# adaptivegenome/openge

Hardware: AMD Instinct MI355X
Metric: Mreads/sec sort+dedup (and realign intervals/sec), 1/2/4/8 MI355X (higher is better)
Workload: dtype u8

## Files before the change

include/openge_hip.h:

```cpp
#ifndef OPENGE_HIP_H
#define OPENGE_HIP_H

#include <stddef.h>
#include <stdint.h>

#ifdef __cplusplus
extern "C" {
#endif

typedef enum oge_status {
    OGE_OK = 0,
    OGE_ERR_ARG = -1,
    OGE_ERR_HIP = -2,
    OGE_ERR_LIMIT = -3,
    OGE_ERR_IO = -4
} oge_status;

typedef struct oge_ctx oge_ctx;

int oge_ctx_create(int device, oge_ctx **out);
int oge_device_count(void);
int oge_ctx_set_stream(oge_ctx *ctx, void *stream);
void *oge_ctx_stream(oge_ctx *ctx);
int oge_ctx_sync(oge_ctx *ctx);
// ... 87 lines not shown
                          uint64_t *n_dup_total);
int oge_bgzf_decode_shard(oge_comm *comm, const uint8_t *d_z, uint64_t zbytes, uint64_t own_bytes, const uint8_t **d_recs,
                          const uint64_t **d_off, uint64_t *n, uint8_t *hdr_out, uint64_t hdr_cap, uint64_t *hdr_len);
int oge_mergesort_bgzf_shard(oge_comm *comm, const uint8_t *d_z, uint64_t zbytes, uint64_t own_bytes, const oge_mergesort_opts *o,
                             const uint8_t **d_out, uint64_t *out_bytes, uint64_t *n_reads_total, uint64_t *n_dup_total);
int oge_synth_offsets_range_dev(oge_ctx *ctx, const void *params, uint64_t slot0, uint64_t nslots, uint64_t *d_offs);
int oge_synth_records_range_dev(oge_ctx *ctx, const void *params, uint64_t slot0, uint64_t nslots,
                                const uint64_t *d_offs, uint8_t *d_out);

typedef struct oge_realign_scan_batch {
    const uint8_t *cons;
    uint64_t cons_bytes;
    const uint64_t *cons_off;
    uint32_t n_cons;
    uint32_t n_reads;
    const uint8_t *bases;
    const uint8_t *quals;
    uint64_t read_bytes;
    const uint64_t *read_off;
    const int32_t *pairs;
    uint64_t n_pairs;
} oge_realign_scan_batch;
int oge_realign_scan(oge_ctx *ctx, const oge_realign_scan_batch *batch, int32_t *best_index, int32_t *best_score);

typedef struct oge_realign_opts {
    double lod_threshold;
    double mismatch_threshold;
    int32_t max_records_in_memory;
    int32_t max_isize_for_movement;
    int32_t max_pos_move_allowed;
    int32_t max_reads;
    int32_t no_original_alignment_tags;
    int32_t threads;
} oge_realign_opts;
void oge_realign_opts_init(oge_realign_opts *opts);

typedef struct oge_realign_result oge_realign_result;
int oge_localrealign(oge_ctx *ctx, const char *header_text, uint64_t header_len, const uint8_t *recs,
                     const uint64_t *rec_off, uint64_t n, const char *fasta_path, const char *intervals_path,
                     const oge_realign_opts *opts, oge_realign_result **out);
int oge_localrealign_multi(oge_ctx *const *ctxs, int n_ctx, const char *header_text, uint64_t header_len, const uint8_t *recs,
                           const uint64_t *rec_off, uint64_t n, const char *fasta_path, const char *intervals_path,
                           const oge_realign_opts *opts, oge_realign_result **out);
uint64_t oge_realign_result_count(const oge_realign_result *r);
const uint8_t *oge_realign_result_records(const oge_realign_result *r, uint64_t *bytes_out);
const uint64_t *oge_realign_result_offsets(const oge_realign_result *r);
const char *oge_realign_result_stats(const oge_realign_result *r);
void oge_realign_result_free(oge_realign_result *r);

int oge_synth_finalize(void *params);
uint64_t oge_synth_params_size(void);
int oge_synth_offsets_host(const void *params, uint64_t *offs, int threads);
int oge_synth_records_host(const void *params, const uint64_t *offs, uint8_t *out, int threads);
int oge_synth_header_text(const void *params, char *buf, uint64_t cap, uint64_t *len_out);
typedef struct oge_realign_synth_params {
    uint64_t seed;
    uint32_t n_ref, n_intervals, spacing, read_len, frags_per_interval;
    uint32_t qual_min, qual_max, ins_min, ins_max;
    uint32_t err_ppm, noindel_ppm, gapped_ppm, alt_indel_ppm, dup_ppm, mapq0_ppm, clip_ppm;
    uint32_t lower_ppm, n_ppm, md_ppm, uq_ppm;
} oge_realign_synth_params;
void oge_realign_synth_defaults(oge_realign_synth_params *p);
int oge_synth_realign(const oge_realign_synth_params *p, const char *fasta_path, const char *intervals_path,
                      const char *bam_path, int level, int threads);
int oge_synth_offsets_dev(oge_ctx *ctx, const void *params, uint64_t *d_offs);
int oge_synth_records_dev(oge_ctx *ctx, const void *params, const uint64_t *d_offs, uint8_t *d_out);

typedef struct oge_bam oge_bam;
int oge_bam_read(const char *path, int threads, oge_bam **out);
void oge_bam_free(oge_bam *b);
uint64_t oge_bam_count(const oge_bam *b);
const uint8_t *oge_bam_records(const oge_bam *b, uint64_t *bytes_out);
const uint64_t *oge_bam_offsets(const oge_bam *b);
int32_t oge_bam_n_ref(const oge_bam *b);
int oge_bam_header_text(const oge_bam *b, char *buf, uint64_t cap, uint64_t *len_out);
int oge_bam_markdup_opts(const oge_bam *b, oge_markdup_opts *opts, char **rg_ids_buf, int16_t **rg_lib_buf);
int oge_bam_write(const char *path, const char *header_text, uint64_t header_len, int sort_order,
                  const uint8_t *recs, const uint64_t *offs, uint64_t n, const uint32_t *order,
                  const uint16_t *flags, int level, int threads);

uint64_t oge_bgzf_bound(uint64_t n);
int oge_bgzf_deflate_dev(oge_ctx *ctx, const uint8_t *d_src, uint64_t n, int level, uint8_t *d_dst,
                         uint64_t dst_cap, uint64_t *out_bytes);
int oge_bgzf_deflate(oge_ctx *ctx, const uint8_t *src, uint64_t n, int level, uint8_t *dst, uint64_t dst_cap,
                     uint64_t *out_bytes);
enum { OGE_DEFL_FAST = 0, OGE_DEFL_NEAR = 1, OGE_DEFL_SPAN = 2 };
int oge_ctx_set_deflate_search(oge_ctx *ctx, int search);
int oge_ctx_deflate_search(oge_ctx *ctx);
int oge_bgzf_index(const uint8_t *z, uint64_t zbytes, uint64_t *d0, uint64_t *d1, uint64_t *uoff, uint32_t *crc,
                   uint64_t cap, uint64_t *nblk);
int oge_bgzf_index_dev(oge_ctx *ctx, const uint8_t *d_z, uint64_t zbytes, uint64_t *d_d0, uint64_t *d_d1,
                       uint64_t *d_uoff, uint32_t *d_crc, uint64_t cap, uint64_t *nblk);
int oge_bgzf_inflate_dev(oge_ctx *ctx, const uint8_t *d_z, uint64_t zbytes, const uint64_t *d_d0, const uint64_t *d_d1,
                         const uint64_t *d_uoff, const uint32_t *d_crc, uint64_t nblk, uint8_t *d_out);
uint64_t oge_infl_plan(uint64_t nblk, uint64_t lanes, uint64_t budget, uint64_t max_per_lane, int balanced,
                       uint64_t *sizes, uint64_t cap);
int oge_bgzf_inflate(oge_ctx *ctx, const uint8_t *z, uint64_t zbytes, uint8_t *out, uint64_t out_cap,
                     uint64_t *out_bytes);
int oge_bam_record_offsets_dev(oge_ctx *ctx, const uint8_t *d_stream, uint64_t rec_base, uint64_t end, int32_t n_ref,
                               uint64_t *d_off, uint64_t cap, uint64_t *n_out);
int oge_fix_bins_dev(oge_ctx *ctx, uint8_t *d_recs, const uint64_t *d_off, uint64_t n);
int oge_drop_flagged_dev(oge_ctx *ctx, const uint8_t *d_recs, const uint64_t *d_off, uint64_t n, uint16_t flag_mask,
                         uint8_t *d_out, uint64_t *d_out_off, uint64_t *n_out);

int oge_bai_build_dev(oge_ctx *ctx, const uint8_t *d_recs, const uint64_t *d_off, uint64_t n, int32_t n_ref,
                      uint64_t stream_base, const uint64_t *d_uoff, const uint64_t *d_cstart, uint64_t nblk,
                      const uint8_t **d_bai, uint64_t *bai_bytes);
int oge_bai_build(oge_ctx *ctx, const uint8_t *recs, uint64_t rec_bytes, const uint64_t *rec_off, uint64_t n,
                  int32_t n_ref, uint64_t stream_base, const uint64_t *uoff, const uint64_t *cstart, uint64_t nblk,
                  uint8_t *out, uint64_t cap, uint64_t *bai_bytes);
int oge_bam_index_dev(oge_ctx *ctx, const uint8_t *d_z, uint64_t zbytes, const uint8_t **d_bai, uint64_t *bai_bytes);
int oge_ctx_last_bai(oge_ctx *ctx, const uint8_t **d_bai, uint64_t *bai_bytes);

typedef struct oge_bai oge_bai;
int oge_bai_open(oge_ctx *ctx, const uint8_t *bai, uint64_t bytes, int32_t n_ref_expected, oge_bai **out);
void oge_bai_close(oge_bai *bai);
struct oge_region;
int oge_bai_query_dev(oge_ctx *ctx, const oge_bai *bai, const struct oge_region *regions, uint64_t n_regions, int32_t widen,
                      const uint64_t **d_ranges, uint64_t *n_ranges);
int oge_bai_query(oge_ctx *ctx, const oge_bai *bai, const struct oge_region *regions, uint64_t n_regions, int32_t widen,
                  uint64_t *out, uint64_t cap, uint64_t *n_ranges);
int oge_bam_decode_ranges_dev(oge_ctx *ctx, const uint8_t *d_z, uint64_t zbytes, const uint64_t *span_z,
                              const uint64_t *span_file, uint64_t n_spans, const uint64_t *d_ranges, uint64_t n_ranges,
                              int32_t n_ref, uint8_t **d_recs, uint64_t **d_off, uint64_t *n, uint64_t *rec_bytes);

typedef struct oge_bam_stats {
    uint64_t reads, mapped, forward, reverse, failed_qc, duplicates, paired, proper_pair, read1, read2, both_mapped,
        singletons;
    int32_t sorted;
    int32_t pad0;
    uint64_t n_insert, insert_sum, insert_mid_lo, insert_mid_hi;
    uint64_t n_lengths;
} oge_bam_stats;
enum { OGE_STATS_INSERTS = 1, OGE_STATS_LENGTHS = 2 };
int oge_stats_dev(oge_ctx *ctx, const uint8_t *d_recs, const uint64_t *d_off, uint64_t n, uint32_t want,
                  oge_bam_stats *stats, const uint32_t **d_len, const uint64_t **d_len_count);
int oge_stats(oge_ctx *ctx, const uint8_t *recs, uint64_t rec_bytes, const uint64_t *rec_off, uint64_t n, uint32_t want,
              oge_bam_stats *stats, uint32_t *len_out, uint64_t *len_count_out, uint64_t cap);
int oge_coverage_layout(int32_t n_ref, const int32_t *ref_len, int32_t binsize, uint64_t *base);
int oge_coverage_dev(oge_ctx *ctx, const uint8_t *d_recs, const uint64_t *d_off, uint64_t n, int32_t n_ref,
                     const int32_t *ref_len, int32_t binsize, const uint32_t **d_bins, uint64_t *n_skipped,
                     int32_t *overflow);
int oge_coverage(oge_ctx *ctx, const uint8_t *recs, uint64_t rec_bytes, const uint64_t *rec_off, uint64_t n,
                 int32_t n_ref, const int32_t *ref_len, int32_t binsize, uint32_t *bins_out, uint64_t cap,
                 uint64_t *n_skipped, int32_t *overflow);
int oge_bam_stats_dev(oge_ctx *ctx, const uint8_t *d_z, uint64_t zbytes, uint32_t want, oge_bam_stats *stats,
                      const uint32_t **d_len, const uint64_t **d_len_count);
int oge_bam_coverage_dev(oge_ctx *ctx, const uint8_t *d_z, uint64_t zbytes, int32_t binsize, const uint32_t **d_bins,
                         uint64_t *n_bins, uint64_t *n_skipped, int32_t *overflow);
int oge_bam_count_dev(oge_ctx *ctx, const uint8_t *d_z, uint64_t zbytes, uint64_t *n_reads);
int oge_ctx_last_refs(oge_ctx *ctx, int32_t *n_ref, const char **names, uint64_t *names_bytes, const int32_t **ref_len);

typedef struct oge_compare_region {
    int32_t left_ref, left_pos, right_ref, right_pos;
} oge_compare_region;
typedef struct oge_compare_result {
    uint64_t n_ref, n_other, common, additions, deletions, diff_entries, hard_runs;
} oge_compare_result;
enum { OGE_COMPARE_DIFF = 1 };
int oge_compare_dev(oge_ctx *ctx, const uint8_t *d_recs_a, const uint64_t *d_off_a, uint64_t n_a, const uint8_t *d_recs_b,
                    const uint64_t *d_off_b, uint64_t n_b, int32_t n_ref, const oge_compare_region *region, uint32_t want,
                    int debug_hash_bits, oge_compare_result *result, const uint8_t **d_diff, uint64_t *diff_bytes);
int oge_compare(oge_ctx *ctx, const uint8_t *recs_a, uint64_t rec_bytes_a, const uint64_t *rec_off_a, uint64_t n_a,
                const uint8_t *recs_b, uint64_t rec_bytes_b, const uint64_t *rec_off_b, uint64_t n_b, int32_t n_ref,
                const oge_compare_region *region, uint32_t want, int debug_hash_bits, oge_compare_result *result,
                uint8_t *diff_out, uint64_t cap, uint64_t *diff_bytes);
// ... 59 lines not shown
```

openge_amd/csrc/bgzf.hip:

```cpp
#include <hip/hip_runtime.h>

#include <cstdint>
#include <cstdlib>
#include <cstring>
#include <string>
#include <vector>

#include "bam_layout.h"
#include "oge_ctx.h"
#include "records.h"
#include "bgzf_dev.h"

namespace {

using namespace oge_bgzf;
constexpr int kT = 512;
constexpr int kSeg = 64;
constexpr int kSub = kT * kSeg;
constexpr int kNSub = 2;
constexpr int kNSeg = kT * kNSub;
constexpr int kHashBits = 12;
constexpr int kLit = 286, kDist = 30, kCl = 19;
constexpr int kFreq = kLit + kDist;
constexpr int kHdrWords = 144;
// ... 1093 lines not shown
            for (int b = 0; b < 4; ++b)
                if (s0 + 4 * k + b < len) v |= (uint32_t)s[s0 + 4 * k + b] << (8 * b);
            w[k] = v;
        }
    }
}

#ifndef OGE_EMIT_MPRE
#define OGE_EMIT_MPRE 8
#endif
constexpr int kMPre = OGE_EMIT_MPRE;
__device__ __forceinline__ void seg_tokens(const uint32_t *mp, uint32_t nm, uint32_t (&m)[kMPre]) {
    const uint32_t last = nm ? nm - 1 : 0;
#pragma unroll
    for (int k = 0; k < kMPre; ++k) m[k] = mp[(uint64_t)min((uint32_t)k, last) * kNSeg];
}

__device__ __forceinline__ uint32_t seg_bits(const uint32_t (&w)[16], uint64_t lm, uint32_t nm, const uint32_t *mp,
                                             const uint32_t (&m)[kMPre], const uint32_t *ct, const uint32_t *dist) {
    uint32_t bits = 0;
#pragma unroll
    for (int g = 0; g < 4; ++g) {
        uint32_t c[16];
#pragma unroll
        for (int i = 0; i < 16; ++i) c[i] = ct[(w[4 * g + (i >> 2)] >> (8 * (i & 3))) & 0xff];
#pragma unroll
        for (int i = 0; i < 16; ++i) bits += (lm >> (16 * g + i)) & 1 ? c[i] >> 24 : 0u;
    }
#pragma unroll
    for (int k = 0; k < kMPre; ++k)
        if ((uint32_t)k < nm) bits += match_bits(m[k], ct, dist);
    for (uint32_t k = kMPre; k < nm; ++k) bits += match_bits(mp[(uint64_t)k * kNSeg], ct, dist);
    return bits;
}

__device__ __forceinline__ void seg_emit(const uint32_t (&w)[16], uint64_t lm, uint32_t nm, const uint32_t *mp,
                                         uint32_t (&m)[kMPre], const uint32_t *ct, const uint32_t *dist, uint32_t *img,
                                         uint32_t bit) {
    uint32_t k = 0, cur = m[0], moff = nm ? (cur >> 23) : 64u;
    uint32_t lc, dv, dn;
    auto look = [&](uint32_t tok) {
        lc = ct[256 + ((tok >> 15) & 255)];
        dist_bits((tok & 0x7fff) + 1, dist, dv, dn);
    };
    look(cur);
    LdsBits bw;
    bw.init(img, bit);
#pragma unroll
    for (int g = 0; g < 4; ++g) {
        uint32_t c[16];
#pragma unroll
        for (int i = 0; i < 16; ++i) c[i] = ct[(w[4 * g + (i >> 2)] >> (8 * (i & 3))) & 0xff];
#pragma unroll
        for (int i0 = 0; i0 < 16; i0 += 2) {
            const int i = 16 * g + i0;
            const uint32_t a = (lm >> i) & 1 ? c[i0] : 0u, b = (lm >> (i + 1)) & 1 ? c[i0 + 1] : 0u;
            bw.put((a & 0xffffff) | ((b & 0xffffff) << (a >> 24)), (a >> 24) + (b >> 24));
            if (((uint32_t)i | 1u) == (moff | 1u)) {
#if OGE_EXP == 8
                ++k;
#pragma unroll
                for (int q = 0; q + 1 < kMPre; ++q) m[q] = m[q + 1];
                moff = k < nm && k < (uint32_t)kMPre ? m[0] >> 23 : 64u;
#else
                bw.put(lc & 0xffffff, lc >> 24);
                bw.put(dv, dn);
                ++k;
#pragma unroll
                for (int q = 0; q + 1 < kMPre; ++q) m[q] = m[q + 1];
                if (k < nm) {
                    cur = k < (uint32_t)kMPre ? m[0] : mp[(uint64_t)k * kNSeg];
                    moff = cur >> 23;
                    look(cur);
                } else {
                    moff = 64;
                }
#endif
            }
        }
    }
    bw.finish();
}

__global__ void __launch_bounds__(kT, 4) k_defl_emit(const uint8_t *__restrict__ src, uint64_t n, uint64_t blk0,
                                                     const uint64_t *__restrict__ lmask, const uint8_t *__restrict__ nmatch,
                                                     const uint32_t *__restrict__ mlist, const DeflTab *__restrict__ tabs,
                                                     const uint32_t *__restrict__ zpow, const uint32_t *__restrict__ offs,
                                                     const uint64_t *__restrict__ cbase, uint8_t *__restrict__ dst) {
    __shared__ __align__(16) uint32_t img[kSlot / 4 + 4];
    __shared__ uint32_t ct[512], dist[kDist];
    __shared__ uint32_t scan[kNSeg];
    __shared__ uint32_t wsum[kT / 64];
    __shared__ uint32_t crctab[4][256];
    __shared__ uint32_t zp[17][32];
    __shared__ uint32_t zl[32][16];
    __shared__ uint32_t crcs[kT / 64];
    __shared__ uint32_t sh_crc;
    const int t = threadIdx.x, lane = t & 63, wv = t >> 6;
    const uint64_t blk = blk0 + blockIdx.x;
    const uint64_t start = blk * kPay;
    const uint32_t len = (uint32_t)min<uint64_t>(kPay, n - start);
    const uint8_t *s = src + start;
    const DeflTab &T = tabs[blockIdx.x];
    const uint32_t total = T.total, stored = T.stored, hb = T.hdr_bits;
    for (int i = t; i < 512; i += kT) ct[i] = ct_entry(i, T.lit);
    for (int i = t; i < kDist; i += kT) dist[i] = T.dist[i];
    crc_setup<kT>(crctab, zp, zpow, t);
    for (int i = t; i < 32 * 16; i += kT) zl[i >> 4][i & 15] = zpow[17 * 32 + i];
    for (uint32_t i = t; i < (total + 15) / 16; i += kT) ((uint4 *)img)[i] = make_uint4(0, 0, 0, 0);
    __syncthreads();
    {
        const uint32_t c = crc_global512x4l(s, len, crctab, zl, zp, crcs, t);
        if (t == 0) sh_crc = c;
    }
    const uint32_t bsize = total - 1;
    if (stored) {
        for (uint32_t i = t; i < len; i += kT) ((uint8_t *)img)[23 + i] = s[i];
    } else {
        const uint32_t s0a = t * kSeg, s0b = kSub + t * kSeg;
        const uint64_t sga = (uint64_t)blockIdx.x * kNSeg + t, sgb = sga + kT;
        const uint64_t lma = s0a < len ? lmask[sga] : 0, lmb = s0b < len ? lmask[sgb] : 0;
        const uint32_t nma = s0a < len ? nmatch[sga] : 0, nmb = s0b < len ? nmatch[sgb] : 0;
        const uint32_t *mpa = mlist + ((uint64_t)blockIdx.x * kMaxM) * kNSeg + t, *mpb = mpa + kT;
        uint32_t ca, cb;
        {
            uint32_t w[16], m[kMPre];
            seg_load(s, s0a, len, w);
            seg_tokens(mpa, nma, m);
            ca = seg_bits(w, lma, nma, mpa, m, ct, dist);
            seg_load(s, s0b, len, w);
            seg_tokens(mpb, nmb, m);
            cb = seg_bits(w, lmb, nmb, mpb, m, ct, dist);
        }
        scan[t] = ca;
        scan[kT + t] = cb;
        __syncthreads();
        {
            const uint32_t a = scan[2 * t], b = scan[2 * t + 1];
            uint32_t x = a + b, inc = x;
#pragma unroll
            for (int o = 1; o < 64; o <<= 1) {
                const uint32_t y = __shfl_up(inc, o);
                if (lane >= o) inc += y;
            }
            if (lane == 63) wsum[wv] = inc;
            __syncthreads();
            uint32_t pre = 0;
            for (int q = 0; q < wv; ++q) pre += wsum[q];
            const uint32_t ex = pre + inc - x;
            __syncthreads();
            scan[2 * t] = ex;
            scan[2 * t + 1] = ex + a;
        }
        __syncthreads();
        for (uint32_t i = t; i < (hb + 31) / 32; i += kT) {
            const uint32_t v = T.hdr[i];
            atomicOr(img + 4 + i, v << 16);
            if (v >> 16) atomicOr(img + 5 + i, v >> 16);
        }
        {
            uint32_t w[16], m[kMPre];
            if (ca) {
                seg_load(s, s0a, len, w);
                seg_tokens(mpa, nma, m);
                seg_emit(w, lma, nma, mpa, m, ct, dist, img, 144 + hb + scan[t]);
            }
            if (cb) {
                seg_load(s, s0b, len, w);
                seg_tokens(mpb, nmb, m);
                seg_emit(w, lmb, nmb, mpb, m, ct, dist, img, 144 + hb + scan[kT + t]);
            }
        }
        if (t == kT - 1) {
            const uint32_t body_end = 144 + hb + scan[kNSeg - 1] + cb;
            LdsBits bw;
            bw.init(img, body_end);
            const uint32_t c = T.lit[256];
            bw.put(c & 0xffff, c >> 16);
            bw.finish();
        }
    }
    __syncthreads();
    uint8_t *ib = (uint8_t *)img;
    if (t == 0) {
        img[0] = 0x04088b1fu;
        img[1] = 0;
        img[2] = 0x0006ff00u;
        img[3] = 0x00024342u;
        ib[16] = (uint8_t)bsize, ib[17] = (uint8_t)(bsize >> 8);
        if (stored) {
            ib[18] = 1;
            ib[19] = (uint8_t)len, ib[20] = (uint8_t)(len >> 8);
            ib[21] = (uint8_t)~len, ib[22] = (uint8_t)(~len >> 8);
        }
        const uint32_t q = total - 8;
        for (int b = 0; b < 4; ++b) ib[q + b] = (uint8_t)(sh_crc >> (8 * b)), ib[q + 4 + b] = (uint8_t)(len >> (8 * b));
    }
    __syncthreads();
    uint8_t *D = dst + *cbase + offs[blockIdx.x];
    const uint32_t sh = (uint32_t)((uintptr_t)D & 3);
    OGE_G uint32_t *A = (OGE_G uint32_t *)((uintptr_t)D & ~(uintptr_t)3);
    const uint32_t nwords = (total + sh + 3) / 4;
    for (uint32_t g = t; g < nwords; g += kT) {
        const int32_t r0 = (int32_t)(4 * g) - (int32_t)sh;
        if (r0 >= 0 && r0 + 4 <= (int32_t)total) {
            A[g] = ld32(img, (uint32_t)r0);
        } else {
            for (int i = 0; i < 4; ++i) {
                const int32_t r = r0 + i;
                if (r >= 0 && r < (int32_t)total) ((OGE_G uint8_t *)(A + g))[i] = ib[r];
            }
        }
    }
}

constexpr uint32_t kMaxChunk = 16384, kPer = kMaxChunk / 1024;
__global__ void __launch_bounds__(1024) k_scan_chunk(const uint32_t *__restrict__ in, uint32_t n, uint32_t *__restrict__ out) {
    __shared__ uint32_t ws[16];
    const uint32_t t = threadIdx.x, lane = t & 63, w = t >> 6;
    uint32_t a[kPer], v = 0;
#pragma unroll
    for (uint32_t i = 0; i < kPer; ++i) {
        a[i] = kPer * t + i < n ? in[kPer * t + i] : 0;
        v += a[i];
    }
    uint32_t x = v;
#pragma unroll
    for (int d = 1; d < 64; d <<= 1) {
        const uint32_t y = __shfl_up(x, d, 64);
        if (lane >= (uint32_t)d) x += y;
    }
    if (lane == 63) ws[w] = x;
    __syncthreads();
    if (t < 16) {
        uint32_t s = ws[t], z = s;
        for (int d = 1; d < 16; d <<= 1) {
            const uint32_t y = __shfl_up(z, d, 16);
            if ((t & 15) >= (uint32_t)d) z += y;
        }
        ws[t] = z - s;
    }
    __syncthreads();
    uint32_t excl = ws[w] + x - v;
#pragma unroll
    for (uint32_t i = 0; i < kPer; ++i) {
        if (kPer * t + i < n) out[kPer * t + i] = excl;
        excl += a[i];
    }
}

__global__ void k_defl_advance(uint64_t *base, uint64_t *cbase, const uint32_t *offs, const uint32_t *sizes, uint32_t nb) {
    if (threadIdx.x == 0 && blockIdx.x == 0) {
        const uint64_t b = *base;
        *cbase = b;
        *base = b + (uint64_t)offs[nb - 1] + sizes[nb - 1];
    }
}

__global__ void k_fix_bins(uint8_t *__restrict__ recs, const uint64_t *__restrict__ off, uint64_t n) {
    const uint64_t i = (uint64_t)blockIdx.x * blockDim.x + threadIdx.x;
    if (i >= n) return;
    uint8_t *r = recs + off[i];
    oge_wr_u16(r + OGE_OFF_BIN, oge_rec_bin(r));
}

}


extern "C" uint64_t oge_bgzf_bound(uint64_t n) { return ((n + kPay - 1) / kPay) * (uint64_t)kSlot; }

extern "C" int oge_bgzf_deflate_dev(oge_ctx *ctx, const uint8_t *d_src, uint64_t n, int level, uint8_t *d_dst,
                                    uint64_t dst_cap, uint64_t *out_bytes) {
    if (!ctx) return oge_fail(nullptr, OGE_ERR_ARG, "null ctx");
    if (!out_bytes || (n && (!d_src || !d_dst))) return oge_fail(ctx, OGE_ERR_ARG, "null buffer");
    if (level < 0 || level > 9) return oge_fail(ctx, OGE_ERR_ARG, "level must be 0..9");
    const int depth = level >= 9 ? 32 : level == 8 ? 8 : 1, lazy = level >= 8 ? 1 : 0;
    const int search = level == 0 ? OGE_DEFL_FAST : ctx->deflate_search;
    if (dst_cap < oge_bgzf_bound(n)) return oge_fail(ctx, OGE_ERR_ARG, "dst_cap < oge_bgzf_bound(n)");
    OgeCall call(ctx, false);
    *out_bytes = 0;
    if (!n) return OGE_OK;
    const uint64_t nblk = (n + kPay - 1) / kPay;
    const int ncu = ctx->cu_count();
#ifndef OGE_DEFL_STREAMS
#define OGE_DEFL_STREAMS 3
#endif
#ifndef OGE_DEFL_CHUNK
#define OGE_DEFL_CHUNK kMaxChunk
#endif
    static_assert(OGE_DEFL_CHUNK <= kMaxChunk, "k_scan_chunk bound");
    constexpr uint64_t kPerPay = (uint64_t)kNSeg * 8 + kNSeg + (uint64_t)kMaxM * kNSeg * 4 + kFreq * 4 + sizeof(DeflTab) + 8;
    const int S0 = nblk > 4096 ? OGE_DEFL_STREAMS : 1;
    uint64_t chunk = std::min<uint64_t>(nblk, OGE_DEFL_CHUNK);
    if (chunk > 4096) {
        size_t fr = 0, tot = 0;
        if (hipMemGetInfo(&fr, &tot) != hipSuccess) fr = 0;
        uint64_t held = 0;
        for (int s = 0; s < 3; ++s) {
            const auto it = ctx->bufs.find("defl_mlist" + std::to_string(s));
            if (it != ctx->bufs.end()) held += it->second.cap / ((uint64_t)kMaxM * kNSeg * 4) * kPerPay;
        }
        while (chunk > 4096 && (uint64_t)S0 * chunk * kPerPay > (fr + held) / 4) chunk = std::max<uint64_t>(4096, chunk / 2);
    }
    static_assert(OGE_DEFL_STREAMS >= 1 && OGE_DEFL_STREAMS <= 3, "deflate: 1-3 streams");
    const int S = nblk > chunk ? OGE_DEFL_STREAMS : 1;
    struct Bufs {
        uint64_t *lmask, *cbase;
        uint32_t *mlist, *freq, *sizes, *offs;
        uint8_t *nmatch;
        DeflTab *tabs;
        hipStream_t st;
    } B[3];
    for (int s = 0; s < S; ++s) {
        const std::string x = std::to_string(s);
        B[s].lmask = (uint64_t *)ctx->ws(("defl_lmask" + x).c_str(), chunk * kNSeg * 8);
        B[s].nmatch = (uint8_t *)ctx->ws(("defl_nmatch" + x).c_str(), chunk * kNSeg);
        B[s].mlist = (uint32_t *)ctx->ws(("defl_mlist" + x).c_str(), chunk * kMaxM * kNSeg * 4);
        B[s].freq = (uint32_t *)ctx->ws(("defl_freq" + x).c_str(), chunk * kFreq * 4);
        B[s].tabs = (DeflTab *)ctx->ws(("defl_tabs" + x).c_str(), chunk * sizeof(DeflTab));
        B[s].sizes = (uint32_t *)ctx->ws(("defl_sizes" + x).c_str(), chunk * 4 + 16);
        B[s].offs = (uint32_t *)ctx->ws(("defl_offs" + x).c_str(), chunk * 4 + 16);
        B[s].cbase = (uint64_t *)ctx->ws(("defl_cbase" + x).c_str(), 16);
        B[s].st = S == 1 ? ctx->stream : ctx->side_stream(s);
        if (!B[s].lmask || !B[s].nmatch || !B[s].mlist || !B[s].freq || !B[s].tabs || !B[s].sizes || !B[s].offs ||
            !B[s].cbase || !B[s].st)
            return OGE_ERR_HIP;
    }
    uint32_t *zpow = (uint32_t *)ctx->ws("defl_zpow", (17 * 32 + 32 * 16) * 4);
    uint64_t *base = (uint64_t *)ctx->ws("defl_base", 16);
    if (!zpow || !base) return OGE_ERR_HIP;
    static struct {
        uint32_t z[17][32], zl[32][16];
    } zh = [] {
        decltype(zh) v;
        crc_zpow(v.z);
        crc_zlane<16>(v.z, 128, &v.zl[0][0]);
        return v;
    }();
    OGE_HIP_TRY(ctx, hipMemcpyAsync(zpow, &zh, sizeof(zh), hipMemcpyHostToDevice, ctx->stream));
    OGE_HIP_TRY(ctx, hipMemsetAsync(base, 0, 8, ctx->stream));
    OgeStage stage(ctx, "bgzf_deflate");
    hipEvent_t ev[4];
    for (auto &e : ev) OGE_HIP_TRY(ctx, hipEventCreateWithFlags(&e, hipEventDisableTiming));
    struct Evs {
        hipEvent_t *e;
        ~Evs() {
            for (int i = 0; i < 4; ++i) hipEventDestroy(e[i]);
        }
    } evs{ev};
    OGE_HIP_TRY(ctx, hipEventRecord(ev[3], ctx->stream));
    for (int s = 0; s < S; ++s)
        if (B[s].st != ctx->stream) OGE_HIP_TRY(ctx, hipStreamWaitEvent(B[s].st, ev[3], 0));
    uint64_t k = 0;
    for (uint64_t b0 = 0; b0 < nblk; b0 += chunk, ++k) {
        const uint32_t nb = (uint32_t)std::min(chunk, nblk - b0);
        Bufs &u = B[k % S];
        const uint32_t pg = (uint32_t)std::min<uint64_t>(nb, (uint64_t)ncu);
#define OGE_PARSE_X(C, N, S) \
    k_defl_parse_x<C, N, S><<<pg, kTP, 0, u.st>>>(d_src, n, b0, nb, u.lmask, u.nmatch, u.mlist, u.freq, depth, lazy)
        if (search == OGE_DEFL_FAST && depth > 1)
            k_defl_parse<true><<<pg, kTP, 0, u.st>>>(d_src, n, b0, nb, u.lmask, u.nmatch, u.mlist, u.freq, depth, lazy);
        else if (search == OGE_DEFL_FAST)
            k_defl_parse<false><<<pg, kTP, 0, u.st>>>(d_src, n, b0, nb, u.lmask, u.nmatch, u.mlist, u.freq, 1, 0);
        else if (search == OGE_DEFL_NEAR)
            depth > 1 ? OGE_PARSE_X(true, true, false) : OGE_PARSE_X(false, true, false);
        else if (search == OGE_DEFL_SPAN)
            depth > 1 ? OGE_PARSE_X(true, false, true) : OGE_PARSE_X(false, false, true);
        else
            depth > 1 ? OGE_PARSE_X(true, true, true) : OGE_PARSE_X(false, true, true);
#undef OGE_PARSE_X
        OGE_LAUNCH_CHECK(ctx);
        k_defl_huff<<<nb, 64, 0, u.st>>>(u.freq, u.tabs, n, b0, level, u.sizes);
        OGE_LAUNCH_CHECK(ctx);
        k_scan_chunk<<<1, 1024, 0, u.st>>>(u.sizes, nb, u.offs);
        OGE_LAUNCH_CHECK(ctx);
        if (k) OGE_HIP_TRY(ctx, hipStreamWaitEvent(u.st, ev[(k - 1) % S], 0));
        k_defl_advance<<<1, 64, 0, u.st>>>(base, u.cbase, u.offs, u.sizes, nb);
        OGE_LAUNCH_CHECK(ctx);
        OGE_HIP_TRY(ctx, hipEventRecord(ev[k % S], u.st));
        k_defl_emit<<<nb, kT, 0, u.st>>>(d_src, n, b0, u.lmask, u.nmatch, u.mlist, u.tabs, zpow, u.offs, u.cbase, d_dst);
        OGE_LAUNCH_CHECK(ctx);
    }
    if (S > 1) {
        for (int s = 0; s < S; ++s) {
            OGE_HIP_TRY(ctx, hipEventRecord(ev[s], B[s].st));
            OGE_HIP_TRY(ctx, hipStreamWaitEvent(ctx->stream, ev[s], 0));
        }
    }
    stage.end();
    uint64_t total = 0;
    OGE_HIP_TRY(ctx, hipMemcpyAsync(&total, base, 8, hipMemcpyDeviceToHost, ctx->stream));
    OGE_HIP_TRY(ctx, hipStreamSynchronize(ctx->stream));
    *out_bytes = total;
    return OGE_OK;
}

extern "C" int oge_bgzf_deflate(oge_ctx *ctx, const uint8_t *src, uint64_t n, int level, uint8_t *dst, uint64_t dst_cap,
                                uint64_t *out_bytes) {
    if (!ctx) return oge_fail(nullptr, OGE_ERR_ARG, "null ctx");
    if (!out_bytes || (n && (!src || !dst))) return oge_fail(ctx, OGE_ERR_ARG, "null buffer");
    hipSetDevice(ctx->device);
    *out_bytes = 0;
    if (!n) return OGE_OK;
    const uint64_t bound = oge_bgzf_bound(n);
    uint8_t *ds = (uint8_t *)ctx->ws("defl_hsrc", n + 16);
    uint8_t *dd = (uint8_t *)ctx->ws("defl_hdst", bound);
    if (!ds || !dd) return OGE_ERR_HIP;
    OGE_HIP_TRY(ctx, hipMemcpyAsync(ds, src, n, hipMemcpyHostToDevice, ctx->stream));
    uint64_t got = 0;
    int rc = oge_bgzf_deflate_dev(ctx, ds, n, level, dd, bound, &got);
    if (rc) return rc;
    if (got > dst_cap) return oge_fail(ctx, OGE_ERR_ARG, "dst_cap too small for the compressed stream");
    OGE_HIP_TRY(ctx, hipMemcpyAsync(dst, dd, got, hipMemcpyDeviceToHost, ctx->stream));
    OGE_HIP_TRY(ctx, hipStreamSynchronize(ctx->stream));
    *out_bytes = got;
    return OGE_OK;
}

extern "C" int oge_fix_bins_dev(oge_ctx *ctx, uint8_t *d_recs, const uint64_t *d_off, uint64_t n) {
    if (!ctx) return oge_fail(nullptr, OGE_ERR_ARG, "null ctx");
    hipSetDevice(ctx->device);
    if (!n) return OGE_OK;
    k_fix_bins<<<oge_ceil_div(n, 256), 256, 0, ctx->stream>>>(d_recs, d_off, n);
    OGE_LAUNCH_CHECK(ctx);
    return OGE_OK;
}
```

openge_amd/lib.py:

```python
from __future__ import annotations

import contextlib
import ctypes as C
import os
from pathlib import Path

import numpy as np

PKG = Path(__file__).resolve().parent
LIB_PATH = Path(os.environ["OGE_LIB"]) if os.environ.get("OGE_LIB") else PKG / "libopenge_hip.so"

MAX_REF = 64
DEFLATE_SEARCH = ("fast", "near", "span", "near+span")


class SynthParams(C.Structure):

    _fields_ = [
        ("seed", C.c_uint64), ("n_pairs", C.c_uint64), ("n_ref", C.c_uint32), ("read_len", C.c_uint32),
        ("ins_min", C.c_uint32), ("ins_max", C.c_uint32), ("dup_ppm", C.c_uint32), ("inter_ppm", C.c_uint32),
        ("munmap_ppm", C.c_uint32), ("clip_ppm", C.c_uint32), ("n_rg", C.c_uint32), ("qual_min", C.c_uint32),
        ("qual_max", C.c_uint32), ("shuffle", C.c_uint32),
        ("ref_len", C.c_uint64 * MAX_REF), ("ref_cum", C.c_uint64 * (MAX_REF + 1)),
    ]
# ... 182 lines not shown
    L = C.CDLL(str(LIB_PATH))
    vp, u64, i32, u32 = C.c_void_p, C.c_uint64, C.c_int32, C.c_uint32
    sig = {
        "oge_ctx_create": (C.c_int, [C.c_int, C.POINTER(vp)]),
        "oge_ctx_set_stream": (C.c_int, [vp, vp]),
        "oge_ctx_stream": (vp, [vp]),
        "oge_ctx_sync": (C.c_int, [vp]),
        "oge_ctx_destroy": (None, [vp]),
        "oge_last_error": (C.c_char_p, [vp]),
        "oge_ctx_timing": (C.c_int, [vp, C.c_char_p, C.POINTER(C.c_double)]),
        "oge_ctx_counter": (C.c_int, [vp, C.c_char_p, C.POINTER(u64)]),
        "oge_mergesort_reserve": (C.c_int, [vp, u64, C.POINTER(vp), C.POINTER(vp), C.POINTER(u64)]),
        "oge_version": (C.c_char_p, []),
        "oge_sort_coord": (C.c_int, [vp, vp, u64, vp, u64, i32, vp]),
        "oge_sort_coord_dev": (C.c_int, [vp, vp, vp, u64, i32, vp]),
        "oge_gather_records_dev": (C.c_int, [vp, vp, vp, vp, u64, vp, vp]),
        "oge_radix_sort_pairs_dev": (C.c_int, [vp, vp, vp, vp, vp, u64, u64, C.POINTER(C.c_int)]),
        "oge_exclusive_scan_dev": (C.c_int, [vp, vp, vp, u64, C.c_int]),
        "oge_markdup": (C.c_int, [vp, vp, u64, vp, u64, vp, vp, C.POINTER(u64)]),
        "oge_markdup_dev": (C.c_int, [vp, vp, vp, u64, vp, vp, C.c_int, C.POINTER(u64)]),
        "oge_sort_markdup_dev": (C.c_int, [vp, vp, vp, u64, vp, vp, vp, vp, C.POINTER(u64)]),
        "oge_synth_finalize": (C.c_int, [vp]),
        "oge_synth_params_size": (u64, []),
        "oge_synth_offsets_host": (C.c_int, [vp, vp, C.c_int]),
        "oge_synth_records_host": (C.c_int, [vp, vp, vp, C.c_int]),
        "oge_synth_header_text": (C.c_int, [vp, vp, u64, C.POINTER(u64)]),
        "oge_synth_offsets_dev": (C.c_int, [vp, vp, vp]),
        "oge_synth_records_dev": (C.c_int, [vp, vp, vp, vp]),
        "oge_bam_read": (C.c_int, [C.c_char_p, C.c_int, C.POINTER(vp)]),
        "oge_bam_free": (None, [vp]),
        "oge_bam_count": (u64, [vp]),
        "oge_bam_records": (vp, [vp, C.POINTER(u64)]),
        "oge_bam_offsets": (vp, [vp]),
        "oge_bam_n_ref": (i32, [vp]),
        "oge_bam_header_text": (C.c_int, [vp, vp, u64, C.POINTER(u64)]),
        "oge_bam_markdup_opts": (C.c_int, [vp, vp, C.POINTER(vp), C.POINTER(vp)]),
        "oge_bam_write": (C.c_int, [C.c_char_p, C.c_char_p, u64, C.c_int, vp, vp, u64, vp, vp, C.c_int, C.c_int]),
        "oge_realign_scan": (C.c_int, [vp, vp, vp, vp]),
        "oge_sort_markdup_chunked": (C.c_int, [vp, vp, vp, u64, i32, vp, u64, vp, vp, C.POINTER(u64), C.POINTER(u64),
                                               C.POINTER(u64)]),
        "oge_mem_info": (C.c_int, [vp, C.POINTER(u64), C.POINTER(u64)]),
        "oge_device_count": (C.c_int, []),
        "oge_comm_unique_id_bytes": (u64, []),
        "oge_comm_unique_id": (C.c_int, [vp, u64]),
        "oge_comm_init_rank": (C.c_int, [vp, C.c_int, C.c_int, vp, C.POINTER(vp)]),
        "oge_comm_init_rank_mode": (C.c_int, [vp, C.c_int, C.c_int, vp, C.c_char_p, C.POINTER(vp)]),
        "oge_comm_stats_json": (C.c_int64, [vp, C.c_char_p, u64]),
        "oge_comm_init": (C.c_int, [vp, C.c_int, vp]),
        "oge_comm_destroy": (None, [vp]),
        "oge_comm_rank": (C.c_int, [vp]),
        "oge_comm_size": (C.c_int, [vp]),
        "oge_comm_transport": (C.c_char_p, [vp]),
        "oge_mergesort_bgzf_host": (C.c_int, [vp, vp, u64, vp, vp, u64, C.POINTER(u64), C.POINTER(u64), C.POINTER(u64)]),
        "oge_mergesort_bgzf_dist": (C.c_int, [vp, vp, u64, vp, C.POINTER(vp), C.POINTER(u64), C.POINTER(u64),
                                              C.POINTER(u64)]),
        "oge_sort_markdup_dist": (C.c_int, [vp, vp, vp, u64, i32, C.c_int, vp, C.POINTER(vp), C.POINTER(vp), C.POINTER(u64),
                                            C.POINTER(u64)]),
        "oge_mergesort_bgzf_shard": (C.c_int, [vp, vp, u64, u64, vp, C.POINTER(vp), C.POINTER(u64), C.POINTER(u64),
                                               C.POINTER(u64)]),
        "oge_bgzf_decode_shard": (C.c_int, [vp, vp, u64, u64, C.POINTER(vp), C.POINTER(vp), C.POINTER(u64), vp, u64,
                                            C.POINTER(u64)]),
        "oge_synth_offsets_range_dev": (C.c_int, [vp, vp, u64, u64, vp]),
        "oge_synth_records_range_dev": (C.c_int, [vp, vp, u64, u64, vp, vp]),
        "oge_dev_alloc": (C.c_int, [vp, u64, C.POINTER(vp)]),
        "oge_dev_free": (C.c_int, [vp, vp]),
        "oge_memcpy": (C.c_int, [vp, vp, vp, u64, C.c_int]),
        "oge_host_alloc": (C.c_int, [vp, u64, C.POINTER(vp)]),
        "oge_ctx_set_pool": (C.c_int, [vp, C.c_int]),
        "oge_ctx_set_deflate_search": (C.c_int, [vp, C.c_int]),
        "oge_ctx_deflate_search": (C.c_int, [vp]),
        "oge_host_free": (C.c_int, [vp, vp]),
        "oge_realign_opts_init": (None, [vp]),
        "oge_localrealign": (C.c_int, [vp, C.c_char_p, u64, vp, vp, u64, C.c_char_p, C.c_char_p, vp, C.POINTER(vp)]),
        "oge_localrealign_multi": (C.c_int, [vp, C.c_int, C.c_char_p, u64, vp, vp, u64, C.c_char_p, C.c_char_p, vp,
                                             C.POINTER(vp)]),
        "oge_realign_result_count": (u64, [vp]),
        "oge_realign_result_records": (vp, [vp, C.POINTER(u64)]),
        "oge_realign_result_offsets": (vp, [vp]),
        "oge_realign_result_stats": (C.c_char_p, [vp]),
        "oge_realign_result_free": (None, [vp]),
        "oge_realign_synth_defaults": (None, [vp]),
        "oge_synth_realign": (C.c_int, [vp, C.c_char_p, C.c_char_p, C.c_char_p, C.c_int, C.c_int]),
        "oge_bgzf_bound": (u64, [u64]),
        "oge_bgzf_deflate_dev": (C.c_int, [vp, vp, u64, C.c_int, vp, u64, C.POINTER(u64)]),
        "oge_bgzf_deflate": (C.c_int, [vp, vp, u64, C.c_int, vp, u64, C.POINTER(u64)]),
        "oge_fix_bins_dev": (C.c_int, [vp, vp, vp, u64]),
        "oge_bgzf_index": (C.c_int, [vp, u64, vp, vp, vp, vp, u64, C.POINTER(u64)]),
        "oge_bgzf_inflate_dev": (C.c_int, [vp, vp, u64, vp, vp, vp, vp, u64, vp]),
        "oge_bgzf_inflate": (C.c_int, [vp, vp, u64, vp, u64, C.POINTER(u64)]),
        "oge_infl_plan": (u64, [u64, u64, u64, u64, C.c_int, vp, u64]),
        "oge_bam_record_offsets_dev": (C.c_int, [vp, vp, u64, u64, i32, vp, u64, C.POINTER(u64)]),
        "oge_drop_flagged_dev": (C.c_int, [vp, vp, vp, u64, C.c_uint16, vp, vp, C.POINTER(u64)]),
        "oge_filter_opts_init": (None, [vp]),
        "oge_parse_region": (C.c_int, [C.c_char_p, C.c_char_p, i32, vp, vp]),
        "oge_filter_records_dev": (C.c_int, [vp, vp, vp, u64, vp, vp, vp, C.POINTER(u64)]),
        "oge_bai_open": (C.c_int, [vp, vp, u64, i32, C.POINTER(vp)]),
        "oge_bai_close": (None, [vp]),
        "oge_bai_query_dev": (C.c_int, [vp, vp, vp, u64, i32, C.POINTER(vp), C.POINTER(u64)]),
        "oge_bai_query": (C.c_int, [vp, vp, vp, u64, i32, vp, u64, C.POINTER(u64)]),
        "oge_bam_decode_ranges_dev": (C.c_int, [vp, vp, u64, vp, vp, u64, vp, u64, i32, C.POINTER(vp), C.POINTER(vp), C.POINTER(u64),
                                                C.POINTER(u64)]),
        "oge_filter_regions_dev": (C.c_int, [vp, vp, vp, u64, vp, vp, u64, vp, vp, C.POINTER(u64)]),
        "oge_sort_name_dev": (C.c_int, [vp, vp, vp, u64, vp]),
        "oge_sort_name": (C.c_int, [vp, vp, u64, vp, u64, vp]),
        "oge_bgzf_index_dev": (C.c_int, [vp, vp, u64, vp, vp, vp, vp, u64, C.POINTER(u64)]),
        "oge_bai_build_dev": (C.c_int, [vp, vp, vp, u64, i32, u64, vp, vp, u64, C.POINTER(vp), C.POINTER(u64)]),
        "oge_bai_build": (C.c_int, [vp, vp, u64, vp, u64, i32, u64, vp, vp, u64, vp, u64, C.POINTER(u64)]),
        "oge_bam_index_dev": (C.c_int, [vp, vp, u64, C.POINTER(vp), C.POINTER(u64)]),
        "oge_ctx_last_bai": (C.c_int, [vp, C.POINTER(vp), C.POINTER(u64)]),
        "oge_stats_dev": (C.c_int, [vp, vp, vp, u64, u32, vp, C.POINTER(vp), C.POINTER(vp)]),
        "oge_stats": (C.c_int, [vp, vp, u64, vp, u64, u32, vp, vp, vp, u64]),
        "oge_compare_dev": (C.c_int, [vp, vp, vp, u64, vp, vp, u64, i32, vp, u32, C.c_int, vp, C.POINTER(vp), C.POINTER(u64)]),
        "oge_compare": (C.c_int, [vp, vp, u64, vp, u64, vp, u64, vp, u64, i32, vp, u32, C.c_int, vp, vp, u64, C.POINTER(u64)]),
        "oge_coverage_layout": (C.c_int, [i32, vp, i32, vp]),
        "oge_coverage_dev": (C.c_int, [vp, vp, vp, u64, i32, vp, i32, C.POINTER(vp), C.POINTER(u64), C.POINTER(i32)]),
        "oge_coverage": (C.c_int, [vp, vp, u64, vp, u64, i32, vp, i32, vp, u64, C.POINTER(u64), C.POINTER(i32)]),
        "oge_bam_stats_dev": (C.c_int, [vp, vp, u64, u32, vp, C.POINTER(vp), C.POINTER(vp)]),
        "oge_bam_coverage_dev": (C.c_int, [vp, vp, u64, i32, C.POINTER(vp), C.POINTER(u64), C.POINTER(u64), C.POINTER(i32)]),
        "oge_bam_count_dev": (C.c_int, [vp, vp, u64, C.POINTER(u64)]),
        "oge_ctx_last_refs": (C.c_int, [vp, C.POINTER(i32), C.POINTER(vp), C.POINTER(u64), C.POINTER(vp)]),
        "oge_text_size_dev": (C.c_int, [vp, vp, vp, u64, vp, vp, vp, C.POINTER(u64), C.POINTER(u64)]),
        "oge_text_emit_dev": (C.c_int, [vp, vp, vp, vp, u64, u64, vp, vp, u64]),
        "oge_text_host_line": (C.c_int, [vp, u64, vp, vp, u64, C.POINTER(u64)]),
        "oge_text_format": (C.c_int, [vp, vp, u64, vp, u64, vp, vp, u64, C.POINTER(u64)]),
        "oge_sam_header": (C.c_int, [vp, u64, C.POINTER(u64), C.POINTER(u64)]),
        "oge_sam_lines_dev": (C.c_int, [vp, vp, u64, u64, vp, u64, C.POINTER(u64)]),
        "oge_sam_size_dev": (C.c_int, [vp, vp, vp, u64, vp, vp, vp, vp, C.POINTER(u64), C.POINTER(u64)]),
        "oge_sam_emit_dev": (C.c_int, [vp, vp, vp, vp, u64, u64, vp, vp, u64]),
        "oge_sam_host_record": (C.c_int, [vp, u64, vp, vp, u64, C.POINTER(u64)]),
        "oge_sam_parse": (C.c_int, [vp, vp, u64, C.POINTER(u64), C.POINTER(vp), C.POINTER(u64), C.POINTER(vp), C.POINTER(u64), C.POINTER(vp)]),
        "oge_mergesort_opts_init": (None, [vp]),
        "oge_mergesort_bgzf_dev": (C.c_int, [vp, vp, u64, vp, C.POINTER(vp), C.POINTER(u64), C.POINTER(u64),
                                             C.POINTER(u64)]),
    }
    for name, (res, args) in sig.items():
        f = getattr(L, name, None)
        if f is None:
            continue
        f.restype, f.argtypes = res, args
    _lib = L
    return L


def filter_opts(**over) -> FilterOpts:
    o = FilterOpts()
    lib().oge_filter_opts_init(C.byref(o))
    for k, v in over.items():
        setattr(o, k, v)
    return o


def parse_region(region: str, refs: list[tuple[str, int]], opts: FilterOpts | None = None) -> FilterOpts:
    o = opts if opts is not None else filter_opts()
    names = b"".join(nm.encode() + b"\0" for nm, _ in refs)
    lens = np.array([ln for _, ln in refs] or [0], dtype=np.int64)
    check(lib().oge_parse_region(region.encode(), names, len(refs), _ptr(lens), C.byref(o)))
    return o


def infl_plan(nblk: int, lanes: int, budget: int, max_per_lane: int = 0, balanced: bool = False) -> list[int]:
    n = int(lib().oge_infl_plan(nblk, lanes, budget, max_per_lane, int(balanced), None, 0))
    sizes = np.zeros(max(n, 1), dtype=np.uint64)
    lib().oge_infl_plan(nblk, lanes, budget, max_per_lane, int(balanced), _ptr(sizes), n)
    return [int(x) for x in sizes[:n]]


# ... 753 lines not shown
```

Measured before the change: 322.4.

## Split deflate emit into small-LDS and large-slot kernels for higher occupancy

The BGZF emit kernel is templated on its LDS image capacity. Blocks whose compressed size fits a 46 KiB cap go to a small instance that aliases the CRC tables onto the image buffer, which lets three workgroups fit per CU. Oversized blocks are listed by the scan kernel and handled by a persistent large-slot instance launched over a grid of at most twice the CU count. The aim is to raise occupancy in the emit stage, at the cost of a second launch, extra syncs, and a big-block index buffer.

```diff
diff --git a/include/openge_hip.h b/include/openge_hip.h
--- a/include/openge_hip.h
+++ b/include/openge_hip.h
@@ -193,6 +193,7 @@
 uint64_t oge_bgzf_bound(uint64_t n);
 int oge_bgzf_deflate_dev(oge_ctx *ctx, const uint8_t *d_src, uint64_t n, int level, uint8_t *d_dst,
                          uint64_t dst_cap, uint64_t *out_bytes);
+uint32_t oge_defl_emit_cap(void);
 int oge_bgzf_deflate(oge_ctx *ctx, const uint8_t *src, uint64_t n, int level, uint8_t *dst, uint64_t dst_cap,
                      uint64_t *out_bytes);
 enum { OGE_DEFL_FAST = 0, OGE_DEFL_NEAR = 1, OGE_DEFL_SPAN = 2 };
diff --git a/openge_amd/csrc/bgzf.hip b/openge_amd/csrc/bgzf.hip
--- a/openge_amd/csrc/bgzf.hip
+++ b/openge_amd/csrc/bgzf.hip
@@ -1199,46 +1199,72 @@
     bw.finish();
 }
 
-__global__ void __launch_bounds__(kT, 4) k_defl_emit(const uint8_t *__restrict__ src, uint64_t n, uint64_t blk0,
-                                                     const uint64_t *__restrict__ lmask, const uint8_t *__restrict__ nmatch,
-                                                     const uint32_t *__restrict__ mlist, const DeflTab *__restrict__ tabs,
-                                                     const uint32_t *__restrict__ zpow, const uint32_t *__restrict__ offs,
-                                                     const uint64_t *__restrict__ cbase, uint8_t *__restrict__ dst) {
-    __shared__ __align__(16) uint32_t img[kSlot / 4 + 4];
+struct EmitCrc {
+    uint32_t crctab[4][256];
+    uint32_t zp[17][32];
+    uint32_t zl[32][16];
+    uint32_t crcs[kT / 64];
+};
+constexpr uint32_t kLdsGranule = 1280;
+constexpr uint32_t kLdsCu = 163840;
+constexpr uint32_t kEmitFixed = (512 + kDist + kNSeg + kT / 64 + 2) * 4;
+constexpr uint32_t emit_lds(uint32_t cap) { return (cap + 16 + kEmitFixed + kLdsGranule - 1) / kLdsGranule * kLdsGranule; }
+#ifndef OGE_EMIT_SMALL_CAP
+#define OGE_EMIT_SMALL_CAP (46 * 1024)
+#endif
+constexpr uint32_t kEmitSmallCap = OGE_EMIT_SMALL_CAP;
+static_assert(kEmitSmallCap % 1024 == 0 && 3 * emit_lds(kEmitSmallCap) <= kLdsCu && 3 * emit_lds(kEmitSmallCap + 1024) > kLdsCu,
+              "small emit instance: three workgroups per CU, and no larger cap does");
+static_assert(sizeof(EmitCrc) <= kEmitSmallCap, "the CRC tables alias the image");
+
+template <uint32_t CAP>
+__device__ __forceinline__ void emit_block(const uint32_t bi, const uint8_t *__restrict__ src, uint64_t n, uint64_t blk0,
+                                           const uint64_t *__restrict__ lmask, const uint8_t *__restrict__ nmatch,
+                                           const uint32_t *__restrict__ mlist, const DeflTab *__restrict__ tabs,
+                                           const uint32_t *__restrict__ zpow, const uint32_t *__restrict__ offs,
+                                           const uint64_t *__restrict__ cbase, uint8_t *__restrict__ dst) {
+    constexpr bool kSmall = CAP < kSlot;
+    const DeflTab &T = tabs[bi];
+    const uint32_t total = T.total, stored = T.stored, hb = T.hdr_bits;
+    __shared__ __align__(16) uint32_t img[CAP / 4 + 4];
     __shared__ uint32_t ct[512], dist[kDist];
     __shared__ uint32_t scan[kNSeg];
     __shared__ uint32_t wsum[kT / 64];
-    __shared__ uint32_t crctab[4][256];
-    __shared__ uint32_t zp[17][32];
-    __shared__ uint32_t zl[32][16];
-    __shared__ uint32_t crcs[kT / 64];
+    __shared__ __align__(16) uint32_t crc_own[kSmall ? 1 : sizeof(EmitCrc) / 4];
     __shared__ uint32_t sh_crc;
-    const int t = threadIdx.x, lane = t & 63, wv = t >> 6;
-    const uint64_t blk = blk0 + blockIdx.x;
+    EmitCrc &C = *(EmitCrc *)(kSmall ? img : crc_own);
+    int tid = threadIdx.x;
+    asm volatile("" : "+v"(tid));
+    const int t = tid, lane = t & 63, wv = t >> 6;
+    const uint64_t blk = blk0 + bi;
     const uint64_t start = blk * kPay;
     const uint32_t len = (uint32_t)min<uint64_t>(kPay, n - start);
     const uint8_t *s = src + start;
-    const DeflTab &T = tabs[blockIdx.x];
-    const uint32_t total = T.total, stored = T.stored, hb = T.hdr_bits;
     for (int i = t; i < 512; i += kT) ct[i] = ct_entry(i, T.lit);
     for (int i = t; i < kDist; i += kT) dist[i] = T.dist[i];
-    crc_setup<kT>(crctab, zp, zpow, t);
-    for (int i = t; i < 32 * 16; i += kT) zl[i >> 4][i & 15] = zpow[17 * 32 + i];
-    for (uint32_t i = t; i < (total + 15) / 16; i += kT) ((uint4 *)img)[i] = make_uint4(0, 0, 0, 0);
+    crc_setup<kT>(C.crctab, C.zp, zpow, t);
+    for (int i = t; i < 32 * 16; i += kT) C.zl[i >> 4][i & 15] = zpow[17 * 32 + i];
+    if (!kSmall)
+        for (uint32_t i = t; i < (total + 15) / 16; i += kT) ((uint4 *)img)[i] = make_uint4(0, 0, 0, 0);
     __syncthreads();
     {
-        const uint32_t c = crc_global512x4l(s, len, crctab, zl, zp, crcs, t);
+        const uint32_t c = crc_global512x4l(s, len, C.crctab, C.zl, C.zp, C.crcs, t);
         if (t == 0) sh_crc = c;
+    }
+    if (kSmall) {
+        __syncthreads();
+        for (uint32_t i = t; i < (total + 15) / 16; i += kT) ((uint4 *)img)[i] = make_uint4(0, 0, 0, 0);
+        if (stored) __syncthreads();
     }
     const uint32_t bsize = total - 1;
     if (stored) {
         for (uint32_t i = t; i < len; i += kT) ((uint8_t *)img)[23 + i] = s[i];
     } else {
         const uint32_t s0a = t * kSeg, s0b = kSub + t * kSeg;
-        const uint64_t sga = (uint64_t)blockIdx.x * kNSeg + t, sgb = sga + kT;
+        const uint64_t sga = (uint64_t)bi * kNSeg + t, sgb = sga + kT;
         const uint64_t lma = s0a < len ? lmask[sga] : 0, lmb = s0b < len ? lmask[sgb] : 0;
         const uint32_t nma = s0a < len ? nmatch[sga] : 0, nmb = s0b < len ? nmatch[sgb] : 0;
-        const uint32_t *mpa = mlist + ((uint64_t)blockIdx.x * kMaxM) * kNSeg + t, *mpb = mpa + kT;
+        const uint32_t *mpa = mlist + ((uint64_t)bi * kMaxM) * kNSeg + t, *mpb = mpa + kT;
         uint32_t ca, cb;
         {
             uint32_t w[16], m[kMPre];
@@ -1283,9 +1309,12 @@
                 seg_emit(w, lma, nma, mpa, m, ct, dist, img, 144 + hb + scan[t]);
             }
             if (cb) {
+                uint32_t tb = t;
+                asm volatile("" : "+v"(tb));
+                const uint64_t lm2 = lmask[(uint64_t)bi * kNSeg + kT + tb];
                 seg_load(s, s0b, len, w);
                 seg_tokens(mpb, nmb, m);
-                seg_emit(w, lmb, nmb, mpb, m, ct, dist, img, 144 + hb + scan[kT + t]);
+                seg_emit(w, lm2, nmb, mpb, m, ct, dist, img, 144 + hb + scan[kT + t]);
             }
         }
         if (t == kT - 1) {
@@ -1314,7 +1343,7 @@
         for (int b = 0; b < 4; ++b) ib[q + b] = (uint8_t)(sh_crc >> (8 * b)), ib[q + 4 + b] = (uint8_t)(len >> (8 * b));
     }
     __syncthreads();
-    uint8_t *D = dst + *cbase + offs[blockIdx.x];
+    uint8_t *D = dst + *cbase + offs[bi];
     const uint32_t sh = (uint32_t)((uintptr_t)D & 3);
     OGE_G uint32_t *A = (OGE_G uint32_t *)((uintptr_t)D & ~(uintptr_t)3);
     const uint32_t nwords = (total + sh + 3) / 4;
@@ -1331,38 +1360,69 @@
     }
 }
 
+template <uint32_t CAP>
+__global__ void __launch_bounds__(kT, CAP < kSlot ? 6 : 4) k_defl_emit(const uint8_t *__restrict__ src, uint64_t n, uint64_t blk0,
+                                                     const uint64_t *__restrict__ lmask, const uint8_t *__restrict__ nmatch,
+                                                     const uint32_t *__restrict__ mlist, const DeflTab *__restrict__ tabs,
+                                                     const uint32_t *__restrict__ zpow, const uint32_t *__restrict__ offs,
+                                                     const uint64_t *__restrict__ cbase, uint8_t *__restrict__ dst, uint32_t cap,
+                                                     const uint32_t *__restrict__ big) {
+    if (CAP < kSlot) {
+        if (tabs[blockIdx.x].total <= cap) emit_block<CAP>(blockIdx.x, src, n, blk0, lmask, nmatch, mlist, tabs, zpow, offs, cbase, dst);
+    } else {
+        const uint32_t nq = big ? big[0] : blockIdx.x + 1;
+#pragma unroll 1
+        for (uint32_t q = blockIdx.x; q < nq; q += gridDim.x) {
+            const uint32_t bi = big ? big[4 + q] : q;
+            if (!big && tabs[bi].total <= cap) break;
+            emit_block<CAP>(bi, src, n, blk0, lmask, nmatch, mlist, tabs, zpow, offs, cbase, dst);
+            __syncthreads();
+        }
+    }
+}
+
 constexpr uint32_t kMaxChunk = 16384, kPer = kMaxChunk / 1024;
-__global__ void __launch_bounds__(1024) k_scan_chunk(const uint32_t *__restrict__ in, uint32_t n, uint32_t *__restrict__ out) {
-    __shared__ uint32_t ws[16];
+__global__ void __launch_bounds__(1024) k_scan_chunk(const uint32_t *__restrict__ in, uint32_t n, uint32_t *__restrict__ out,
+                                                     uint32_t cap, unsigned long long *__restrict__ nsmall,
+                                                     uint32_t *__restrict__ big) {
+    __shared__ uint32_t ws[16], wb[16];
     const uint32_t t = threadIdx.x, lane = t & 63, w = t >> 6;
-    uint32_t a[kPer], v = 0;
+    uint32_t a[kPer], v = 0, nbig = 0, small = 0;
 #pragma unroll
     for (uint32_t i = 0; i < kPer; ++i) {
         a[i] = kPer * t + i < n ? in[kPer * t + i] : 0;
         v += a[i];
-    }
-    uint32_t x = v;
+        small += a[i] && a[i] <= cap;
+        nbig += a[i] > cap;
+    }
+#pragma unroll
+    for (int d = 32; d >= 1; d >>= 1) small += __shfl_xor(small, d, 64);
+    if (lane == 0 && small) atomicAdd(nsmall, (unsigned long long)small);
+    uint32_t x = v, xb = nbig;
 #pragma unroll
     for (int d = 1; d < 64; d <<= 1) {
-        const uint32_t y = __shfl_up(x, d, 64);
-        if (lane >= (uint32_t)d) x += y;
-    }
-    if (lane == 63) ws[w] = x;
+        const uint32_t y = __shfl_up(x, d, 64), yb = __shfl_up(xb, d, 64);
+        if (lane >= (uint32_t)d) x += y, xb += yb;
+    }
+    if (lane == 63) ws[w] = x, wb[w] = xb;
     __syncthreads();
     if (t < 16) {
-        uint32_t s = ws[t], z = s;
+        uint32_t s = ws[t], z = s, sb = wb[t], zb = sb;
         for (int d = 1; d < 16; d <<= 1) {
-            const uint32_t y = __shfl_up(z, d, 16);
-            if ((t & 15) >= (uint32_t)d) z += y;
+            const uint32_t y = __shfl_up(z, d, 16), yb = __shfl_up(zb, d, 16);
+            if ((t & 15) >= (uint32_t)d) z += y, zb += yb;
         }
         ws[t] = z - s;
-    }
-    __syncthreads();
-    uint32_t excl = ws[w] + x - v;
+        wb[t] = zb - sb;
+        if (t == 15) big[0] = zb;
+    }
+    __syncthreads();
+    uint32_t excl = ws[w] + x - v, rank = wb[w] + xb - nbig;
 #pragma unroll
     for (uint32_t i = 0; i < kPer; ++i) {
         if (kPer * t + i < n) out[kPer * t + i] = excl;
         excl += a[i];
+        if (a[i] > cap) big[4 + rank++] = kPer * t + i;
     }
 }
 
@@ -1385,6 +1445,14 @@
 
 
 extern "C" uint64_t oge_bgzf_bound(uint64_t n) { return ((n + kPay - 1) / kPay) * (uint64_t)kSlot; }
+
+extern "C" uint32_t oge_defl_emit_cap(void) { return kEmitSmallCap; }
+
+static uint32_t emit_cap_now() {
+    const char *e = getenv("OGE_DEFL_EMIT_CAP");
+    if (!e || !*e) return kEmitSmallCap;
+    return (uint32_t)std::min<unsigned long long>(strtoull(e, nullptr, 10), kEmitSmallCap);
+}
 
 extern "C" int oge_bgzf_deflate_dev(oge_ctx *ctx, const uint8_t *d_src, uint64_t n, int level, uint8_t *d_dst,
                                     uint64_t dst_cap, uint64_t *out_bytes) {
@@ -1423,7 +1491,7 @@
     const int S = nblk > chunk ? OGE_DEFL_STREAMS : 1;
     struct Bufs {
         uint64_t *lmask, *cbase;
-        uint32_t *mlist, *freq, *sizes, *offs;
+        uint32_t *mlist, *freq, *sizes, *offs, *big;
         uint8_t *nmatch;
         DeflTab *tabs;
         hipStream_t st;
@@ -1438,9 +1506,10 @@
         B[s].sizes = (uint32_t *)ctx->ws(("defl_sizes" + x).c_str(), chunk * 4 + 16);
         B[s].offs = (uint32_t *)ctx->ws(("defl_offs" + x).c_str(), chunk * 4 + 16);
         B[s].cbase = (uint64_t *)ctx->ws(("defl_cbase" + x).c_str(), 16);
+        B[s].big = (uint32_t *)ctx->ws(("defl_big" + x).c_str(), chunk * 4 + 16);
         B[s].st = S == 1 ? ctx->stream : ctx->side_stream(s);
         if (!B[s].lmask || !B[s].nmatch || !B[s].mlist || !B[s].freq || !B[s].tabs || !B[s].sizes || !B[s].offs ||
-            !B[s].cbase || !B[s].st)
+            !B[s].cbase || !B[s].big || !B[s].st)
             return OGE_ERR_HIP;
     }
     uint32_t *zpow = (uint32_t *)ctx->ws("defl_zpow", (17 * 32 + 32 * 16) * 4);
@@ -1455,7 +1524,8 @@
         return v;
     }();
     OGE_HIP_TRY(ctx, hipMemcpyAsync(zpow, &zh, sizeof(zh), hipMemcpyHostToDevice, ctx->stream));
-    OGE_HIP_TRY(ctx, hipMemsetAsync(base, 0, 8, ctx->stream));
+    OGE_HIP_TRY(ctx, hipMemsetAsync(base, 0, 16, ctx->stream));
+    const uint32_t ecap = emit_cap_now();
     OgeStage stage(ctx, "bgzf_deflate");
     hipEvent_t ev[4];
     for (auto &e : ev) OGE_HIP_TRY(ctx, hipEventCreateWithFlags(&e, hipEventDisableTiming));
@@ -1489,13 +1559,21 @@
         OGE_LAUNCH_CHECK(ctx);
         k_defl_huff<<<nb, 64, 0, u.st>>>(u.freq, u.tabs, n, b0, level, u.sizes);
         OGE_LAUNCH_CHECK(ctx);
-        k_scan_chunk<<<1, 1024, 0, u.st>>>(u.sizes, nb, u.offs);
+        k_scan_chunk<<<1, 1024, 0, u.st>>>(u.sizes, nb, u.offs, ecap, (unsigned long long *)(base + 1), u.big);
         OGE_LAUNCH_CHECK(ctx);
         if (k) OGE_HIP_TRY(ctx, hipStreamWaitEvent(u.st, ev[(k - 1) % S], 0));
         k_defl_advance<<<1, 64, 0, u.st>>>(base, u.cbase, u.offs, u.sizes, nb);
         OGE_LAUNCH_CHECK(ctx);
         OGE_HIP_TRY(ctx, hipEventRecord(ev[k % S], u.st));
-        k_defl_emit<<<nb, kT, 0, u.st>>>(d_src, n, b0, u.lmask, u.nmatch, u.mlist, u.tabs, zpow, u.offs, u.cbase, d_dst);
+        if (ecap) {
+            k_defl_emit<kEmitSmallCap><<<nb, kT, 0, u.st>>>(d_src, n, b0, u.lmask, u.nmatch, u.mlist, u.tabs, zpow, u.offs, u.cbase,
+                                                            d_dst, ecap, nullptr);
+            OGE_LAUNCH_CHECK(ctx);
+            k_defl_emit<kSlot><<<std::min<uint32_t>(nb, 2 * (uint32_t)ncu), kT, 0, u.st>>>(d_src, n, b0, u.lmask, u.nmatch, u.mlist, u.tabs,
+                                                                                           zpow, u.offs, u.cbase, d_dst, ecap, u.big);
+        } else {
+            k_defl_emit<kSlot><<<nb, kT, 0, u.st>>>(d_src, n, b0, u.lmask, u.nmatch, u.mlist, u.tabs, zpow, u.offs, u.cbase, d_dst, 0, nullptr);
+        }
         OGE_LAUNCH_CHECK(ctx);
     }
     if (S > 1) {
@@ -1505,10 +1583,16 @@
         }
     }
     stage.end();
-    uint64_t total = 0;
-    OGE_HIP_TRY(ctx, hipMemcpyAsync(&total, base, 8, hipMemcpyDeviceToHost, ctx->stream));
+    uint64_t total[2] = {0, 0};
+    OGE_HIP_TRY(ctx, hipMemcpyAsync(total, base, 16, hipMemcpyDeviceToHost, ctx->stream));
     OGE_HIP_TRY(ctx, hipStreamSynchronize(ctx->stream));
-    *out_bytes = total;
+    *out_bytes = total[0];
+    ctx->counters["defl_emit_small"] += total[1];
+    ctx->counters["defl_emit_big"] += nblk - total[1];
+    static const bool tr = getenv("OGE_TRACE_DEFL") != nullptr;
+    if (tr)
+        fprintf(stderr, "[oge defl] %llu blocks, %llu bytes, emit cap %u: %llu small, %llu big\n", (unsigned long long)nblk,
+                (unsigned long long)total[0], ecap, (unsigned long long)total[1], (unsigned long long)(nblk - total[1]));
     return OGE_OK;
 }
 
diff --git a/openge_amd/lib.py b/openge_amd/lib.py
--- a/openge_amd/lib.py
+++ b/openge_amd/lib.py
@@ -288,6 +288,7 @@
         "oge_realign_synth_defaults": (None, [vp]),
         "oge_synth_realign": (C.c_int, [vp, C.c_char_p, C.c_char_p, C.c_char_p, C.c_int, C.c_int]),
         "oge_bgzf_bound": (u64, [u64]),
+        "oge_defl_emit_cap": (u32, []),
         "oge_bgzf_deflate_dev": (C.c_int, [vp, vp, u64, C.c_int, vp, u64, C.POINTER(u64)]),
         "oge_bgzf_deflate": (C.c_int, [vp, vp, u64, C.c_int, vp, u64, C.POINTER(u64)]),
         "oge_fix_bins_dev": (C.c_int, [vp, vp, vp, u64]),
```

Measured after the change: 328.3, median of 6. 1.02x the previous value.
